# akb825/Cuttlefish

Measured on AMD Instinct MI355X. Metric: Mpixels/s encode, BC7 4096x4096 RGBA8, higher is better.
Workload: dtype u8; 1 GPU; BC7 UNORM Texture::Quality::Normal, one 4096x4096 RGBA8 synthetic photo tile per GPU, resident in HBM; format=BC7, quality=2, blocks_per_launch=1048576, parallelism=surface-per-gpu x1

## Files before the change

cuttlefish_amd/csrc/bc7_encode.hip:

```cpp
#include "cf_device.h"
#include "bc7_packed.h"
#include "bc7_rcp.h"
#include "bc7_roles.h"
#include "bc7_cand.h"

namespace {

#define CF_FRESH_LANE(x) asm volatile("v_mbcnt_lo_u32_b32 %0, -1, 0\n\tv_mbcnt_hi_u32_b32 %0, -1, %0" : "=v"(x))

__device__ __forceinline__ int cf_bperm(int v, uint32_t src)
{
	return __builtin_amdgcn_ds_bpermute((int)(src << 2), v);
}

__device__ const cf_bc7_role_table k_bc7_roles = cf_bc7_make_roles();

__device__ const cf_bc7_cand_table k_bc7_cands = cf_bc7_make_cands();
__device__ const cf_bc7_mask_table k_bc7_masks = cf_bc7_make_masks();

__device__ const cf_bc7_weight_table k_bc7_weights = cf_bc7_make_weights();

__device__ const uint16_t k_part2[64] = CF_BC7_PART2_INIT;

__device__ const uint8_t k_anchor2[64] = {
	15,15,15,15,15,15,15,15, 15,15,15,15,15,15,15,15,
	15, 2, 8, 2, 2, 8, 8,15,  2, 8, 2, 2, 8, 8, 2, 2,
	15,15, 6, 8, 2, 8,15,15,  2, 8, 2, 2, 2,15,15, 6,
	 6, 2, 6, 8,15,15, 2, 2, 15,15,15,15,15, 2, 2,15
};

__device__ const uint32_t k_part3[64] = CF_BC7_PART3_INIT;

__device__ const uint8_t k_anchor3a[64] = {
	 3, 3,15,15, 8, 3,15,15,  8, 8, 6, 6, 6, 5, 3, 3,
	 3, 3, 8,15, 3, 3, 6,10,  5, 8, 8, 6, 8, 5,15,15,
	 8,15, 3, 5, 6,10, 8,15, 15, 3,15, 5,15,15,15,15,
	 3,15, 5, 5, 5, 8, 5,10,  5,10, 8,13,15,12, 3, 3
};

__device__ const uint8_t k_anchor3b[64] = {
	15, 8, 8, 3,15,15, 3, 8, 15,15,15,15,15,15,15, 8,
	15, 8,15, 3,15, 8,15, 8,  3,15, 6,10,15,15,10, 8,
	15, 3,15,10,10, 8, 9,10,  6,15, 8,15, 3, 6, 6, 8,
	15, 3,15,15,15,15,15,15, 15,15,15,15, 3,15,15, 8
};

__device__ __forceinline__ uint32_t part3_mask(uint32_t p3, uint32_t sb)
{
	const uint32_t lo = p3 & 0x55555555u, hi = (p3 >> 1) & 0x55555555u;
	uint32_t x = sb == 0u ? ~(lo | hi) & 0x55555555u : (sb == 1u ? lo & ~hi : (sb == 2u ? hi & ~lo : 0u));
	x = (x | (x >> 1)) & 0x33333333u;
	x = (x | (x >> 2)) & 0x0F0F0F0Fu;
	x = (x | (x >> 4)) & 0x00FF00FFu;
	return (x | (x >> 8)) & 0xFFFFu;
}

struct SubFit {
	uint32_t e0, e1;
	uint32_t q0, q1;
	uint32_t pb;
	uint32_t err;
	uint32_t w[4];
	float nx0[4], nx1[4];
	bool ok;
};

struct Cand {
	uint32_t err, id;
	uint32_t q[6];
	uint32_t pb;
	uint32_t w[4];
	uint32_t w2[4];
};

#define CF_BC7_CAND_WORDS 22
__device__ __forceinline__ void cand_store(uint32_t* slot, const Cand& c)
{
#pragma unroll
	for (int k = 0; k < 6; ++k) slot[k*CF_WG_THREADS] = c.q[k];
	slot[6*CF_WG_THREADS] = c.pb;
#pragma unroll
	for (int k = 0; k < 4; ++k) {
		slot[(7 + k)*CF_WG_THREADS] = c.w[k];
		slot[(11 + k)*CF_WG_THREADS] = c.w2[k];
	}
}

__device__ __forceinline__ uint32_t ub(uint32_t v, int c) { return (v >> (8*c)) & 255u; }
__device__ __forceinline__ float fb(uint32_t v, int c) { return (float)((v >> (8*c)) & 255u); }

__device__ __forceinline__ float clamp255(float x)
{
	return __builtin_amdgcn_fmed3f(x, 0.0f, 255.0f);
}

__device__ const float k_inv_n[17] = {
	__builtin_huge_valf(), 1.0f/1.0f, 1.0f/2.0f, 1.0f/3.0f, 1.0f/4.0f, 1.0f/5.0f, 1.0f/6.0f, 1.0f/7.0f, 1.0f/8.0f,
	1.0f/9.0f, 1.0f/10.0f, 1.0f/11.0f, 1.0f/12.0f, 1.0f/13.0f, 1.0f/14.0f, 1.0f/15.0f, 1.0f/16.0f
};
__device__ __forceinline__ float inv_n(uint32_t n) { return k_inv_n[n < 16u ? n : 16u]; }

// ... 159 lines not shown
}

#ifndef CF_BC7_ABLATE
#define CF_BC7_ABLATE 0
#endif

#ifndef CF_BC7_DIAG
#define CF_BC7_DIAG 0
#endif
#if CF_BC7_DIAG
enum { CF_DIAG_STARTS, CF_DIAG_STARTS_CACHED, CF_DIAG_STARTS_NARROW, CF_DIAG_PERTURB, CF_DIAG_PERTURB_NARROW,
	CF_DIAG_STARTS_NOPB, CF_DIAG_PERTURB_NOPB, CF_DIAG_PERTURB_PPHIT, CF_DIAG_N };
__device__ unsigned long long cf_bc7_diag[CF_DIAG_N];
#define CF_DIAG_COUNT(i, cond) do { uint32_t l_; CF_FRESH_LANE(l_); if (l_ == 0u && (cond)) atomicAdd(&cf_bc7_diag[i], 1ull); } while (0)
#else
#define CF_DIAG_COUNT(i, cond) do { } while (0)
#endif

typedef int cf_int4 __attribute__((ext_vector_type(4)));
template <bool UNITW>
__device__ __forceinline__ void arow_load(const uint32_t* tile, uint32_t boff, uint32_t (&arow)[4])
{
	arow[0] = arow[1] = arow[2] = arow[3] = 0u;
	if (UNITW) {
		uint32_t lane;
		CF_FRESH_LANE(lane);
#pragma unroll
		for (uint32_t r = 0; r < 4u; ++r)
			arow[r] = tile[boff + 4u*r + (lane & 3u)] ^ 0x80808080u;
	}
}

struct LaneFit {
	uint32_t q0, q1, pb, err;
	uint32_t w[4];
};

template <bool UNITW, int NK = 8, int CBSZ = 3>
__device__ __forceinline__ void assign_lsq_lane(const Tex& tx, uint32_t mask, bool m6,
	uint32_t khalf, uint32_t ib, const uint32_t (&yw)[2], uint32_t pp_sum, bool want_lsq, uint32_t fe0, uint32_t fe1, const uint32_t (&arow)[4],
	LaneFit& f, float (&nx0)[4], float (&nx1)[4], float (&hq)[3], bool& ok, uint32_t s01 = 0u, uint32_t s23 = 0u)
{
	constexpr int WBITS = UNITW ? 8 : 7;
	const uint32_t nk = m6 ? 8u : (1u << ib);
	const uint32_t e00 = ub(fe0, 0), e01 = ub(fe0, 1), e02 = ub(fe0, 2), e03 = ub(fe0, 3);
	const uint32_t e10 = ub(fe1, 0), e11 = ub(fe1, 1), e12 = ub(fe1, 2), e13 = ub(fe1, 3);
	uint32_t pal[8], palh[8];
	int base[8];
	uint32_t w03 = 0, w47 = 0;
	const uint32_t* wr = k_bc7_weights.w[weight_row(m6, khalf, ib)];
	w03 = wr[0];
	w47 = NK == 8 ? wr[1] : 0u;
	const uint32_t rsel = tx.rot == 0u ? 0x03020100u : (tx.rot == 1u ? 0x00020103u : (tx.rot == 2u ? 0x01020300u : 0x02030100u));
	const PalLine line = pal_line(__builtin_amdgcn_perm(fe0, fe0, rsel), __builtin_amdgcn_perm(fe1, fe1, rsel));
#pragma unroll
	for (int k = 0; k < NK; ++k) {
		const bool valid = k < 4 || (uint32_t)k < nk;
		const uint32_t w = weight_at(w03, w47, (uint32_t)k);
		const uint32_t iw = 64u - w;
		if (UNITW) {
			pal[k] = pal_at(line, w);
			palh[k] = 0;
			const int B = mfma_entry_base((int)((__builtin_amdgcn_udot4(pal[k], pal[k], 0u, false) << WBITS) | w),
				__builtin_amdgcn_udot4(pal[k], 0x01010101u, 0u, false), WBITS + 1);
			pal[k] ^= 0x80808080u;
			base[k] = valid ? B : CF_BC7_NO_ENTRY;
		} else {
			const uint32_t c0 = (__umul24(iw, e00) + __umul24(w, e10) + 32u) >> 6;
			const uint32_t c1 = (__umul24(iw, e01) + __umul24(w, e11) + 32u) >> 6;
			const uint32_t c2 = (__umul24(iw, e02) + __umul24(w, e12) + 32u) >> 6;
			const uint32_t c3 = (__umul24(iw, e03) + __umul24(w, e13) + 32u) >> 6;
			uint32_t qrg, qba;
			ycc_pairs(c0, c1, c2, c3, qrg, qba);
			pal[k] = pk_mul_u16(qrg, yw[0]);
			palh[k] = pk_mul_u16(qba, yw[1]);
			const uint32_t qq = dot2_u16(pal[k], qrg, dot2_u16(palh[k], qba, 0u));
			const int B = (int)((qq << WBITS) | w);
			base[k] = valid ? B : CF_BC7_NO_ENTRY;
		}
		asm volatile("" : "+v"(base[k]));
	}
	int kfac = -(2 << WBITS);
	asm volatile("" : "+s"(kfac));
	uint32_t err = pp_sum;
	uint32_t wp0 = 0, wp1 = 0, wp2 = 0, wp3 = 0;
#pragma unroll 1
	for (uint32_t r2 = 0; r2 < 4u; r2 += 2u) {
		uint32_t wpair[2];
#pragma unroll
		for (uint32_t h = 0; h < 2u; ++h) {
			const uint32_t r = r2 + h;
			uint32_t raw[4], rawh[4];
			if (UNITW) {
				const uint4 rw = *reinterpret_cast<const uint4*>(tx.tp() + 4u*r);
				raw[0] = rw.x; raw[1] = rw.y; raw[2] = rw.z; raw[3] = rw.w;
				rawh[0] = rawh[1] = rawh[2] = rawh[3] = 0u;
			} else {
				const uint4 ya = *reinterpret_cast<const uint4*>(tx.yc() + 8u*r);
				const uint4 yb = *reinterpret_cast<const uint4*>(tx.yc() + 8u*r + 4u);
				raw[0] = ya.x; raw[1] = ya.z; raw[2] = yb.x; raw[3] = yb.z;
				rawh[0] = ya.y; rawh[1] = ya.w; rawh[2] = yb.y; rawh[3] = yb.w;
			}
			const uint32_t mrow = (mask >> (4u*r)) & 15u;
			uint32_t wrow = 0, krow[4];
			int bestm[4] = {0x7FFFFFFF, 0x7FFFFFFF, 0x7FFFFFFF, 0x7FFFFFFF};
			if (UNITW) {
				const cf_int4 cop = {0, 0, 0, 0};
				const uint32_t aop = r2 == 0u ? (h == 0u ? arow[0] : arow[1]) : (h == 0u ? arow[2] : arow[3]);
#pragma unroll
				for (int k = 0; k < NK; ++k) {
					const cf_int4 d = __builtin_amdgcn_mfma_i32_4x4x4i8((int)aop, (int)pal[k], cop, CBSZ, 0, 0);
					const int v0 = key_min_form(d.x, kfac, base[k]), v1 = key_min_form(d.y, kfac, base[k]);
					const int v2 = key_min_form(d.z, kfac, base[k]), v3 = key_min_form(d.w, kfac, base[k]);
					bestm[0] = v0 < bestm[0] ? v0 : bestm[0]; bestm[1] = v1 < bestm[1] ? v1 : bestm[1];
					bestm[2] = v2 < bestm[2] ? v2 : bestm[2]; bestm[3] = v3 < bestm[3] ? v3 : bestm[3];
				}
			}
#pragma unroll
			for (int j = 0; j < 4; ++j) {
				uint32_t rawj = raw[j];
				if (!UNITW) asm volatile("" : "+v"(rawj), "+v"(wrow));
				uint32_t key;
				{
					int bestk = bestm[j];
					const uint32_t prg = rawj, pba = rawh[j];
#pragma unroll
					for (int k = 0; k < (UNITW ? 0 : NK); ++k) {
						const int dt = (int)dot2_u16(pba, palh[k], dot2_u16(prg, pal[k], 0u));
						const int v = key_min_form(dt, kfac, base[k]);
						bestk = v < bestk ? v : bestk;
					}
					if (NK == 8) {
						const int other = (int)cf_xor1((uint32_t)bestk);
						bestk = (m6 && other < bestk) ? other : bestk;
					}
					key = (uint32_t)bestk;
				}
				key = ((mrow >> j) & 1u) ? key : 0u;
				err += (uint32_t)((int)key >> WBITS);
				if (UNITW) krow[j] = key;
				else wrow |= (key & 127u) << (8*j);
			}
			wpair[h] = UNITW ? key_row_weights(krow[0], krow[1], krow[2], krow[3]) : wrow;
		}
		wp0 = wp2; wp1 = wp3; wp2 = wpair[0]; wp3 = wpair[1];
	}
	f.err = err;
	f.w[0] = wp0; f.w[1] = wp1; f.w[2] = wp2; f.w[3] = wp3;
	uint32_t S = 0, A = 0, B = 0, C = 0, U[4] = {0, 0, 0, 0}, V[4] = {0, 0, 0, 0};
	if (want_lsq) {
#pragma unroll 1
		for (uint32_t r = 0; r < 4u; ++r) {
			const uint32_t wrow = wp0;
			wp0 = wp1; wp1 = wp2; wp2 = wp3; wp3 = wrow;
			uint32_t P[4];
			uint32_t bo = tx.boff;
			asm volatile("" : "+v"(bo));
			planes<true>(tx, *reinterpret_cast<const uint4*>(tx.plan_ + bo + 4u*r), P);
			S = __builtin_amdgcn_udot4(wrow, 0x01010101u, S, false);
			C = __builtin_amdgcn_udot4(wrow, wrow, C, false);
#pragma unroll
			for (int c = 0; c < 4; ++c)
				V[c] = __builtin_amdgcn_udot4(wrow, P[c], V[c], false);
		}
		A = 4096u*(uint32_t)__builtin_popcount(mask) - 128u*S + C;
		B = 64u*S - C;
		U[0] = 64u*(s01 & 0xFFFFu) - V[0]; U[1] = 64u*(s01 >> 16) - V[1];
		U[2] = 64u*(s23 & 0xFFFFu) - V[2]; U[3] = 64u*(s23 >> 16) - V[3];
	}
	const int det = (int)__umul24((uint32_t)__builtin_popcount(mask), C) - (int)__umul24(S, S);
	ok = det > 0;
	const float inv = cf_rcp_ranged(64.0f*(float)(det > 0 ? det : 1));
	const float fA = (float)A, fB = (float)B, fC = (float)C;
#pragma unroll
	for (int c = 0; c < 4; ++c) {
		if ((tx.chmask >> c) & 1u) {
			const float fU = (float)U[c], fV = (float)V[c];
			const float t0 = fB*fV;
			const float n0 = fmaf(fC, fU, -t0);
			const float t1 = fB*fU;
			const float n1 = fmaf(fA, fV, -t1);
			nx0[c] = n0*inv;
			nx1[c] = n1*inv;
		} else {
			nx0[c] = 0.0f;
			nx1[c] = 0.0f;
		}
	}
	hq[0] = fA; hq[1] = fB; hq[2] = fC;
}

__device__ __forceinline__ void refit_window(const float (&xu0)[4], const float (&xu1)[4], const float (&hq)[3],
	uint32_t cb, uint32_t ab, uint32_t pbk, SubFit& f)
{
	const uint32_t S = pbk ? 1u : 0u;
	const uint32_t P0 = f.pb & 1u, P1 = (f.pb >> 1) & 1u;
	const float fA = hq[0], fC = hq[2], fB2 = hq[1] + hq[1];
	const uint32_t tc = cb ? cb + S : 0u, ta = ab ? ab + S : 0u;
	const uint32_t qmaxw = ((1u << cb) - 1u)*0x010101u | (((1u << ab) - 1u) << 24);
	const uint32_t lo0 = f.q0, lo1 = f.q1;
	const uint32_t hi0 = f.q0 ^ qmaxw, hi1 = f.q1 ^ qmaxw;
	uint32_t dw0[3], dw1[3];
	dw0[0] = dequant_word(code_word(((f.q0 | 0x00808080u) - 0x01010101u) & qmaxw, S, P0), tc, ta);
	dw0[1] = f.e0;
	dw0[2] = dequant_word(code_word((f.q0 + 0x01010101u) & qmaxw, S, P0), tc, ta);
	dw1[0] = dequant_word(code_word(((f.q1 | 0x00808080u) - 0x01010101u) & qmaxw, S, P1), tc, ta);
	dw1[1] = f.e1;
	dw1[2] = dequant_word(code_word((f.q1 + 0x01010101u) & qmaxw, S, P1), tc, ta);
	uint32_t pick = 0;
#pragma unroll
	for (int c = 0; c < 4; ++c) {
		const uint32_t bm = 255u << (8*c);
		float dl0[3], dl1[3];
#pragma unroll
		for (int d = 0; d < 3; ++d) {
			dl0[d] = fb(dw0[d], c) - xu0[c];
			dl1[d] = fb(dw1[d], c) - xu1[c];
		}
		dl0[0] = (lo0 & bm) ? dl0[0] : 1.0e18f;
		dl0[2] = (hi0 & bm) ? dl0[2] : 1.0e18f;
		dl1[0] = (lo1 & bm) ? dl1[0] : 1.0e18f;
		dl1[2] = (hi1 & bm) ? dl1[2] : 1.0e18f;
		float best = 3.0e38f;
		uint32_t bi = 0x11u << (8*c);
#pragma unroll
		for (int i = 0; i < 3; ++i) {
			const float d0 = dl0[i];
			float a0 = fA*d0;
			a0 = a0*d0;
			const float cr = fB2*d0;
#pragma unroll
			for (int j = 0; j < 3; ++j) {
				const float d1 = dl1[j];
				float v = fC*d1;
				v = fmaf(v, d1, a0);
				v = fmaf(cr, d1, v);
				const bool take = v < best;
				best = take ? v : best;
				bi = take ? (uint32_t)(i | (j << 4)) << (8*c) : bi;
			}
		}
		pick |= bi;
	}
	const uint32_t nq0 = f.q0 + (pick & 0x03030303u) - 0x01010101u;
	const uint32_t nq1 = f.q1 + ((pick >> 4) & 0x03030303u) - 0x01010101u;
	const uint32_t ne0 = dequant_word(code_word(nq0, S, P0), tc, ta);
	const uint32_t ne1 = dequant_word(code_word(nq1, S, P1), tc, ta);
	f.q0 = nq0; f.q1 = nq1; f.e0 = ne0; f.e1 = ne1;
}

#define CF_BC7_GEO_WORDS 13
// ... 33 lines not shown
		const uint32_t n = (uint32_t)__builtin_popcount(mask);
		uint32_t s[4] = {0, 0, 0, 0};
		uint32_t q00 = 0, q01 = 0, q02 = 0, q03 = 0, q11 = 0, q12 = 0, q13 = 0, q22 = 0, q23 = 0,
			q33 = 0;
		lo = 255u; hi = 0u;
		if (GIVEN && gmode == 3u) {
			uint32_t q[10];
			mom_unpack(gs.W, s, q);
			q00 = q[0]; q01 = q[1]; q02 = q[2]; q03 = q[3]; q11 = q[4]; q12 = q[5]; q13 = q[6]; q22 = q[7]; q23 = q[8]; q33 = q[9];
			lo = gs.lohi & 255u; hi = UNITW ? lohi_hi(gs.lohi) : gs.lohi >> 8;
		} else
#pragma unroll 1
		for (uint32_t r = 0; r < 4u; ++r) {
			uint32_t P[4];
			const uint4 pr = *reinterpret_cast<const uint4*>(tx.pl() + 4u*r);
			planes<true>(tx, pr, P);
			const uint32_t a4 = tx.rot == 0u ? pr.w : (tx.rot == 1u ? pr.x : (tx.rot == 2u ? pr.y : pr.z));
#pragma unroll
			for (int j = 0; j < 4; ++j) {
				const uint32_t a = (a4 >> (8*j)) & 255u;
				lo = a < lo ? a : lo;
				hi = a > hi ? a : hi;
			}
			const uint32_t m4 = bytemask4((mask >> (4u*r)) & 15u);
			const uint32_t M0 = P[0] & m4, M1 = P[1] & m4, M2 = P[2] & m4, M3 = P[3] & m4;
			s[0] = __builtin_amdgcn_udot4(M0, 0x01010101u, s[0], false);
			s[1] = __builtin_amdgcn_udot4(M1, 0x01010101u, s[1], false);
			s[2] = __builtin_amdgcn_udot4(M2, 0x01010101u, s[2], false);
			s[3] = __builtin_amdgcn_udot4(M3, 0x01010101u, s[3], false);
			q00 = __builtin_amdgcn_udot4(M0, P[0], q00, false);
			q01 = __builtin_amdgcn_udot4(M0, P[1], q01, false);
			q02 = __builtin_amdgcn_udot4(M0, P[2], q02, false);
			q03 = __builtin_amdgcn_udot4(M0, P[3], q03, false);
			q11 = __builtin_amdgcn_udot4(M1, P[1], q11, false);
			q12 = __builtin_amdgcn_udot4(M1, P[2], q12, false);
			q13 = __builtin_amdgcn_udot4(M1, P[3], q13, false);
			q22 = __builtin_amdgcn_udot4(M2, P[2], q22, false);
			q23 = __builtin_amdgcn_udot4(M2, P[3], q23, false);
			q33 = __builtin_amdgcn_udot4(M3, P[3], q33, false);
		}
		const float C00 = (float)(int)(__umul24(n, q00) - __umul24(s[0], s[0])), C01 = (float)(int)(__umul24(n, q01) - __umul24(s[0], s[1]));
		const float C02 = (float)(int)(__umul24(n, q02) - __umul24(s[0], s[2])), C03 = (float)(int)(__umul24(n, q03) - __umul24(s[0], s[3]));
		const float C11 = (float)(int)(__umul24(n, q11) - __umul24(s[1], s[1])), C12 = (float)(int)(__umul24(n, q12) - __umul24(s[1], s[2]));
		const float C13 = (float)(int)(__umul24(n, q13) - __umul24(s[1], s[3])), C22 = (float)(int)(__umul24(n, q22) - __umul24(s[2], s[2]));
		const float C23 = (float)(int)(__umul24(n, q23) - __umul24(s[2], s[3])), C33 = (float)(int)(__umul24(n, q33) - __umul24(s[3], s[3]));

		float bestd = C00;
		float v0 = C00, v1 = C01, v2 = C02, v3 = C03;
		if (C11 > bestd) { bestd = C11; v0 = C01; v1 = C11; v2 = C12; v3 = C13; }
		if (C22 > bestd) { bestd = C22; v0 = C02; v1 = C12; v2 = C22; v3 = C23; }
		if (C33 > bestd) { bestd = C33; v0 = C03; v1 = C13; v2 = C23; v3 = C33; }
#pragma unroll
		for (int it = 0; it < 3; ++it) {
			float r0 = C00*v0; r0 = fmaf(C01, v1, r0); r0 = fmaf(C02, v2, r0); r0 = fmaf(C03, v3, r0);
			float r1 = C01*v0; r1 = fmaf(C11, v1, r1); r1 = fmaf(C12, v2, r1); r1 = fmaf(C13, v3, r1);
			float r2 = C02*v0; r2 = fmaf(C12, v1, r2); r2 = fmaf(C22, v2, r2); r2 = fmaf(C23, v3, r2);
			float r3 = C03*v0; r3 = fmaf(C13, v1, r3); r3 = fmaf(C23, v2, r3); r3 = fmaf(C33, v3, r3);
			v0 = r0; v1 = r1; v2 = r2; v3 = r3;
		}
		const float mx = fmaxf(fmaxf(fabsf(v0), fabsf(v1)), fmaxf(fabsf(v2), fabsf(v3)));
#pragma unroll
		for (int c = 0; c < 4; ++c) axis[c] = 0.0f;
		if (mx > 0.0f) {
			const float im = cf_rcp_tested(mx);
			v0 = v0*im; v1 = v1*im; v2 = v2*im; v3 = v3*im;
			float l2 = v0*v0;
			l2 = fmaf(v1, v1, l2);
			l2 = fmaf(v2, v2, l2);
			l2 = fmaf(v3, v3, l2);
			const float is = cf_rcp_ranged(sqrtf(l2));
			axis[0] = v0*is; axis[1] = v1*is; axis[2] = v2*is; axis[3] = v3*is;
		}

		const float in = inv_n(n);
#pragma unroll
		for (int c = 0; c < 4; ++c)
			mean[c] = (float)s[c]*in;
		tmin = 3.0e38f; tmax = -3.0e38f;
#pragma unroll 1
		for (uint32_t r = 0; r < 4u; ++r) {
			const uint4 rw = *reinterpret_cast<const uint4*>(tx.tp() + 4u*r);
			const uint32_t raw[4] = {rw.x, rw.y, rw.z, rw.w};
			const uint32_t mrow = (mask >> (4u*r)) & 15u;
#pragma unroll
			for (int j = 0; j < 4; ++j) {
				const uint32_t p = texel<true>(tx, raw[j]);
				const bool m = (mrow >> j) & 1u;
				float t = axis[0]*(fb(p, 0) - mean[0]);
				t = fmaf(axis[1], fb(p, 1) - mean[1], t);
				t = fmaf(axis[2], fb(p, 2) - mean[2], t);
				t = fmaf(axis[3], fb(p, 3) - mean[3], t);
				tmin = m ? fminf(tmin, t) : tmin;
				tmax = m ? fmaxf(tmax, t) : tmax;
			}
		}
		pp_sum = UNITW ? q00 + q11 + q22 + q33 : ycc_pp_sum(tx, mask, yw);
		if constexpr (UNITW) {
			const uint32_t bias = whole ? lohi_rawsum((GIVEN && gmode == 3u) ? gs.lohi : lohi[tx.boff >> 2])
				: search_bias_part(s[0], s[1], s[2], s[3], n, !(tx.chmask & 8u));
			pp_sum = search_pp_fold(pp_sum, bias);
		}
		s01 = s[0] | (s[1] << 16);
		s23 = s[2] | (s[3] << 16);
		if ((GIVEN ? gmode != 0u : gmode == 1u) && (UNITW ? owner : true)) {
			uint32_t lane;
			CF_FRESH_LANE(lane);
			uint32_t* gc = gbase + lane;
#pragma unroll
			for (int c = 0; c < 4; ++c) {
				gc[c*CF_WG_THREADS] = __float_as_uint(axis[c]);
				gc[(4 + c)*CF_WG_THREADS] = __float_as_uint(mean[c]);
			}
			gc[8*CF_WG_THREADS] = __float_as_uint(tmin);
			gc[9*CF_WG_THREADS] = __float_as_uint(tmax);
			gc[10*CF_WG_THREADS] = lo | (hi << 8);
			gc[11*CF_WG_THREADS] = pp_sum;
		}
	}
	{
		const float d = (tmax - tmin)*frac;
		tmin = tmin + d;
		tmax = tmax - d;
	}
	float x0[4], x1[4];
#pragma unroll
	for (int c = 0; c < 4; ++c) {
		x0[c] = clamp255(fmaf(axis[c], tmin, mean[c]));
		x1[c] = clamp255(fmaf(axis[c], tmax, mean[c]));
	}
	if (scalar) {
		const float flo = (float)lo, fhi = (float)hi;
		const float d = (fhi - flo)*frac;
		x0[0] = 0.0f; x0[1] = 0.0f; x0[2] = 0.0f; x0[3] = clamp255(flo + d);
		x1[0] = 0.0f; x1[1] = 0.0f; x1[2] = 0.0f; x1[3] = clamp255(fhi - d);
	}
	uint32_t geo = cb | (ab << 4) | (pbk << 8) | (ib << 12);
	asm volatile("" : "+v"(geo));
#define G_CB (geo & 15u)
#define G_AB ((geo >> 4) & 15u)
#define G_PBK ((geo >> 8) & 15u)
#define G_IB (geo >> 12)
	SubFit q;
	quantize<UNITW>(x0, x1, G_CB, G_AB, G_PBK, wt, q);
	best.q0 = q.q0; best.q1 = q.q1; best.pb = q.pb;
	bool live;
	float hq[3];
	uint32_t arow[4];
	arow_load<UNITW>(tx.tile_, tx.boff, arow);
	assign_lsq_lane<UNITW, NK, CBSZ>(tx, mask, m6, khalf, G_IB, yw, pp_sum, ITERS > 0u, q.e0, q.e1, arow, best, x0, x1, hq, live, s01, s23);
#pragma unroll 1
	for (uint32_t r = 0; r < ITERS; ++r) {
		LaneFit cur;
		bool ok;
		asm volatile("" : "+v"(geo));
		{
			float c0[4], c1[4];
#pragma unroll
			for (int c = 0; c < 4; ++c) {
				c0[c] = clamp255(x0[c]);
				c1[c] = clamp255(x1[c]);
			}
			quantize<UNITW>(c0, c1, G_CB, G_AB, G_PBK, wt, q);
		}
		if (!(CF_BC7_ABLATE & 8)) refit_window(x0, x1, hq, G_CB, G_AB, G_PBK, q);
		cur.q0 = q.q0; cur.q1 = q.q1; cur.pb = q.pb;
		arow_load<UNITW>(tx.tile_, tx.boff, arow);
		assign_lsq_lane<UNITW, NK, CBSZ>(tx, mask, m6, khalf, G_IB, yw, pp_sum, r + 1u < ITERS, q.e0, q.e1, arow, cur, x0, x1, hq, ok, s01, s23);
		const bool better = live && cur.err < best.err;
		if (better)
			best = cur;
		live = better && ok;
	}
#undef G_CB
#undef G_AB
#undef G_PBK
#undef G_IB
}

__device__ __forceinline__ uint32_t w2i(uint32_t w, uint32_t ib)
{
	return (w*((1u << ib) - 1u) + 32u) >> 6;
}

__device__ __forceinline__ uint4 pack_block_group(const uint32_t* wcol, uint32_t id, uint32_t lane,
	bool pair)
{
	const uint32_t h = lane >> 5, hl = pair ? (lane & 31u) : lane, hbase = pair ? (lane & 32u) : 0u;
	uint32_t mode, part = 0, rot = 0, isel = 0;
	if (id == 0u) mode = 6;
	else if (id < 5u) { mode = 5; rot = id - 1u; }
	else if (id < 13u) { mode = 4; rot = (id - 5u) & 3u; isel = (id - 5u) >> 2; }
	else if (id < 128u) { mode = 1; part = id - 64u; }
	else if (id < 192u) { mode = 3; part = id - 128u; }
	else if (id < 256u) { mode = 0; part = id - 192u; }
	else if (id < 320u) { mode = 2; part = id - 256u; }
	else { mode = 7; part = id - 320u; }
	const uint32_t ns  = (0x21112323u >> (4u*mode)) & 15u;
	const uint32_t pbn = (0x60006664u >> (4u*mode)) & 15u;
	const uint32_t cb  = (0x57757564u >> (4u*mode)) & 15u;
	const uint32_t ab  = (0x57860000u >> (4u*mode)) & 15u;
	const uint32_t pk  = (0x11001021u >> (4u*mode)) & 15u;
	const uint32_t ib  = (0x24222233u >> (4u*mode)) & 15u;
	const uint32_t ib2 = (0x00230000u >> (4u*mode)) & 15u;
	uint32_t ibc = ib, iba = ib2;
	const bool swapsets = mode == 4u && isel != 0u;
	if (swapsets) { ibc = 3u; iba = 2u; }
	const uint32_t p2 = k_part2[part], p3 = k_part3[part];
	uint32_t a1 = 0, a2 = 0;
	if (ns == 2u) a1 = k_anchor2[part];
	else if (ns == 3u) { a1 = k_anchor3a[part]; a2 = k_anchor3b[part]; }

	const uint32_t t = hl & 15u;
	const uint32_t sb = ns == 1u ? 0u : (ns == 2u ? ((p2 >> t) & 1u) : ((p3 >> (2u*t)) & 3u));
	const uint32_t wv = (wcol[(7u + (t >> 2))*CF_WG_THREADS] >> (8u*(t & 3u))) & 255u;
	const uint32_t ws = (wcol[(11u + (t >> 2))*CF_WG_THREADS] >> (8u*(t & 3u))) & 255u;
	uint32_t idxv = w2i(wv, ibc);
	uint32_t idxs = iba ? w2i(ws, iba) : 0u;
	const uint32_t i0 = (uint32_t)cf_bperm((int)idxv, (uint32_t)((int)hbase));
	const uint32_t i1 = (uint32_t)cf_bperm((int)idxv, (uint32_t)((int)(hbase + a1)));
	const uint32_t i2 = (uint32_t)cf_bperm((int)idxv, (uint32_t)((int)(hbase + a2)));
	const uint32_t is0 = (uint32_t)cf_bperm((int)idxs, (uint32_t)((int)hbase));
	const uint32_t sw0 = i0 >> (ibc - 1u);
	const uint32_t sw1 = ns > 1u ? i1 >> (ibc - 1u) : 0u;
	const uint32_t sw2 = ns > 2u ? i2 >> (ibc - 1u) : 0u;
	const uint32_t sws = iba ? is0 >> (iba - 1u) : 0u;
	const uint32_t swmask = sw0 | (sw1 << 1) | (sw2 << 2);
	idxv = ((swmask >> sb) & 1u) ? ((1u << ibc) - 1u) - idxv : idxv;
	idxs = sws ? ((1u << iba) - 1u) - idxs : idxs;

	const uint32_t ne = 2u*ns;
	const uint32_t hdr = mode + 1u + pbn + ((mode == 4u || mode == 5u) ? 2u : 0u) + (mode == 4u ? 1u : 0u);
	const uint32_t base_pb = hdr + ne*(3u*cb + ab);
	const uint32_t npb = pk == 1u ? ne : (pk == 2u ? 2u : 0u);
	const uint32_t baseA = base_pb + npb;
	const uint32_t baseB = baseA + 16u*ib - ns;

	uint32_t w0 = 0, w1 = 0, w2 = 0, w3 = 0;
	const uint32_t npass = pair ? 2u : 1u;
	for (uint32_t pass = 0; pass < npass; ++pass) {
		const uint32_t f = hl + 32u*pass;
		uint32_t val = 0, off = 0;
		bool have = false;
		if (f < 16u) {
			const uint32_t before = (t > 0u ? 1u : 0u) + ((ns >= 2u && t > a1) ? 1u : 0u) +
				((ns == 3u && t > a2) ? 1u : 0u);
			val = swapsets ? idxs : idxv;
			off = baseA + t*ib - before;
			have = true;
		} else if (f < 32u) {
			val = swapsets ? idxv : idxs;
			off = baseB + t*ib2 - (t > 0u ? 1u : 0u);
			have = ib2 != 0u;
		} else if (f < 56u) {
			const uint32_t g = f - 32u;
			const uint32_t ch = g/ne, e = g - ch*ne;
			const uint32_t es = e ^ ((swmask >> (e >> 1)) & 1u);
			const uint32_t qw = wcol[es*CF_WG_THREADS];
			if (ch < 3u) {
				val = (qw >> (8u*ch)) & 255u;
				off = hdr + (ch*ne + e)*cb;
				have = true;
			} else if (ch == 3u && ab) {
				const uint32_t sq = wcol[(4u + ((e ^ sws) & 1u))*CF_WG_THREADS];
				val = (iba ? sq : qw) >> 24;
				off = hdr + 3u*ne*cb + e*ab;
				have = true;
			}
		} else if (f < 62u) {
			const uint32_t e = f - 56u;
			const uint32_t pbw = wcol[6u*CF_WG_THREADS];
			if (pk == 1u && e < ne) {
				val = (pbw >> (e ^ ((swmask >> (e >> 1)) & 1u))) & 1u;
				off = base_pb + e;
				have = true;
			} else if (pk == 2u && e < 2u) {
				val = (pbw >> (2u*e)) & 1u;
				off = base_pb + e;
				have = true;
			}
		} else if (f == 62u) {
			val = (1u << mode) | (part << (mode + 1u)) | (rot << (mode + 1u + pbn)) |
				(isel << (mode + 1u + pbn + 2u));
			if (!(mode == 4u || mode == 5u))
				val = (1u << mode) | (part << (mode + 1u));
			off = 0;
			have = true;
		}
		val = have ? val : 0u;
		const uint32_t wi = off >> 5, sh = off & 31u;
		const unsigned long long vv = (unsigned long long)val << sh;
		const uint32_t lo = (uint32_t)vv, hi = (uint32_t)(vv >> 32);
		w0 |= wi == 0u ? lo : 0u;
		w1 |= wi == 1u ? lo : (wi == 0u ? hi : 0u);
		w2 |= wi == 2u ? lo : (wi == 1u ? hi : 0u);
		w3 |= wi == 3u ? lo : (wi == 2u ? hi : 0u);
	}
	uint4 r;
	r.x = cf_group_or_u32(w0, pair, h);
	r.y = cf_group_or_u32(w1, pair, h);
	r.z = cf_group_or_u32(w2, pair, h);
	r.w = cf_group_or_u32(w3, pair, h);
	return r;
}

struct Moments {
	uint32_t s[4];
	uint32_t q00, q01, q02, q03, q11, q12, q13, q22, q23, q33;
};

#define CF_BC7_MOM_WORDS 10
__device__ __forceinline__ void block_moments_put(const uint32_t* plan, uint32_t* mom, uint32_t t)
{
	const uint32_t b = t >> 4, m = t & 15u;
	if (m >= CF_BC7_MOM_WORDS)
		return;
	const uint32_t ca = m < 4u ? m : (m < 7u ? 0u : (m < 9u ? 1u : 2u));
	const uint32_t cb = m < 4u ? m : (m < 7u ? m - 3u : (m < 9u ? m - 5u : 3u));
	const uint32_t* pb = plan + b*16u;
	const bool opaque = (pb[3] & pb[7] & pb[11] & pb[15]) == 0xFFFFFFFFu;
	uint32_t q = 0, sm = 0;
#pragma unroll
	for (uint32_t r = 0; r < 4u; ++r) {
		const uint32_t A = (opaque && ca == 3u) ? 0u : pb[4u*r + ca], B = (opaque && cb == 3u) ? 0u : pb[4u*r + cb];
		q = __builtin_amdgcn_udot4(A, B, q, false);
		sm = __builtin_amdgcn_udot4(A, 0x01010101u, sm, false);
	}
	mom[b*CF_BC7_MOM_WORDS + m] = m < 4u ? q | (sm << 20) : q;
}

template <bool A4, bool TWO>
__device__ __forceinline__ void moments_rows(const Tex& tx, uint32_t mask1, uint32_t mask2, Moments& a, Moments& b)
{
#pragma unroll
	for (int c = 0; c < 4; ++c) { a.s[c] = 0; b.s[c] = 0; }
	a.q00 = a.q01 = a.q02 = a.q03 = a.q11 = a.q12 = a.q13 = a.q22 = a.q23 = a.q33 = 0;
	b.q00 = b.q01 = b.q02 = b.q03 = b.q11 = b.q12 = b.q13 = b.q22 = b.q23 = b.q33 = 0;
#pragma unroll 1
	for (uint32_t r = 0; r < 4u; ++r) {
		uint32_t P[4];
		planes<false>(tx, *reinterpret_cast<const uint4*>(tx.pl() + 4u*r), P);
#pragma unroll
		for (int k = 0; k < (TWO ? 2 : 1); ++k) {
			Moments& o = k ? b : a;
			const uint32_t m4 = bytemask4(((k ? mask2 : mask1) >> (4u*r)) & 15u);
			const uint32_t M0 = P[0] & m4, M1 = P[1] & m4, M2 = P[2] & m4, M3 = A4 ? P[3] & m4 : 0u;
			o.s[0] = __builtin_amdgcn_udot4(M0, 0x01010101u, o.s[0], false);
			o.s[1] = __builtin_amdgcn_udot4(M1, 0x01010101u, o.s[1], false);
			o.s[2] = __builtin_amdgcn_udot4(M2, 0x01010101u, o.s[2], false);
			if (A4) o.s[3] = __builtin_amdgcn_udot4(M3, 0x01010101u, o.s[3], false);
			o.q00 = __builtin_amdgcn_udot4(M0, P[0], o.q00, false);
			o.q01 = __builtin_amdgcn_udot4(M0, P[1], o.q01, false);
			o.q02 = __builtin_amdgcn_udot4(M0, P[2], o.q02, false);
			if (A4) o.q03 = __builtin_amdgcn_udot4(M0, P[3], o.q03, false);
			o.q11 = __builtin_amdgcn_udot4(M1, P[1], o.q11, false);
			o.q12 = __builtin_amdgcn_udot4(M1, P[2], o.q12, false);
			if (A4) o.q13 = __builtin_amdgcn_udot4(M1, P[3], o.q13, false);
			o.q22 = __builtin_amdgcn_udot4(M2, P[2], o.q22, false);
			if (A4) o.q23 = __builtin_amdgcn_udot4(M2, P[3], o.q23, false);
			if (A4) o.q33 = __builtin_amdgcn_udot4(M3, P[3], o.q33, false);
		}
	}
}

template <bool A4, bool TWO>
__device__ __forceinline__ Moments moments_rest(const uint32_t* tw, const Moments& a, const Moments& b)
{
	Moments o;
	const uint32_t w0 = tw[0], w1 = tw[1], w2 = tw[2], w3 = A4 ? tw[3] : 0u;
#define CF_REST(f, tot) o.f = (tot) - a.f - (TWO ? b.f : 0u)
	CF_REST(s[0], w0 >> 20); CF_REST(s[1], w1 >> 20); CF_REST(s[2], w2 >> 20);
	CF_REST(q00, w0 & 0xFFFFFu); CF_REST(q11, w1 & 0xFFFFFu); CF_REST(q22, w2 & 0xFFFFFu);
// ... 889 lines not shown
```

cuttlefish_amd/csrc/bc7_packed.h:

```cpp
#ifndef CFHIP_BC7_PACKED_H
#define CFHIP_BC7_PACKED_H

#include <stdint.h>

#if defined(__HIPCC__)
#define CF_PK __host__ __device__ __forceinline__
#else
#define CF_PK static inline
#endif
#if defined(__HIP_DEVICE_COMPILE__)
#define CF_PK_MUL24(a, b) __umul24((a), (b))
#else
#define CF_PK_MUL24(a, b) ((a)*(b))
#endif

#if defined(__HIP_DEVICE_COMPILE__)
#define CF_PK_MUL24S(a, b) __mul24((a), (b))
#else
#define CF_PK_MUL24S(a, b) ((a)*(b))
#endif

#define CF_BC7_NO_ENTRY 0x3FFFFFFF
CF_PK int key_min_form(int dt, int m256, int B) { return CF_PK_MUL24S(dt, m256) + B; }


CF_PK int mfma_entry_base(int B, uint32_t sb, int fbits)
{
	return B + (int)(512u << (7 + fbits)) - (int)CF_PK_MUL24(sb, 1u << (7 + fbits));
}

CF_PK uint32_t lohi_pack(uint32_t lohi, uint32_t rawsum) { return lohi | (rawsum << 16); }
CF_PK uint32_t lohi_rawsum(uint32_t w) { return w >> 16; }
CF_PK uint32_t lohi_hi(uint32_t w) { return (w >> 8) & 255u; }
CF_PK uint32_t search_bias_part(uint32_t s0, uint32_t s1, uint32_t s2, uint32_t s3, uint32_t n, bool opaque)
{
	return s0 + s1 + s2 + s3 + (opaque ? CF_PK_MUL24(n, 255u) : 0u);
}
CF_PK uint32_t search_pp_fold(uint32_t pp_sum, uint32_t bias) { return pp_sum - (bias << 8); }

CF_PK uint32_t key_row_weights(uint32_t k0, uint32_t k1, uint32_t k2, uint32_t k3)
{
#if defined(__HIP_DEVICE_COMPILE__)
	return __builtin_amdgcn_perm(k1, k0, 0x0C0C0400u) | __builtin_amdgcn_perm(k3, k2, 0x04000C0Cu);
#else
	return (k0 & 255u) | ((k1 & 255u) << 8) | ((k2 & 255u) << 16) | ((k3 & 255u) << 24);
#endif
}

CF_PK uint32_t dequant1(uint32_t v, uint32_t t)
{
	return CF_PK_MUL24(v, (1u << t) + 1u) >> (2u*t - 8u);
}

CF_PK uint32_t dequant_rgb(uint32_t word, uint32_t t)
{
	const uint32_t c3 = word & 0x00FFFFFFu;
	const uint32_t low = ((1u << (8u - t)) - 1u)*0x010101u;
	return (c3 << (8u - t)) | ((c3 >> (2u*t - 8u)) & low);
}

CF_PK uint32_t dequant_word(uint32_t word, uint32_t tc, uint32_t ta)
{
	const uint32_t coded = (tc ? 0x00FFFFFFu : 0u) | (ta ? 0xFF000000u : 0u);
	return (dequant_rgb(word, tc ? tc : 8u) | (dequant1(word >> 24, ta ? ta : 8u) << 24)) & coded;
}

CF_PK uint32_t code_word(uint32_t qword, uint32_t S, uint32_t P)
{
	return (qword << S) | (P ? 0x01010101u : 0u);
}

CF_PK uint32_t pal_word(uint32_t e0, uint32_t e1, uint32_t w)
{
	const uint32_t iw = 64u - w;
	const uint32_t m = 0x00FF00FFu, half = 0x00200020u;
	const uint32_t rb = CF_PK_MUL24(iw, e0 & m) + CF_PK_MUL24(w, e1 & m) + half;
	const uint32_t ga = CF_PK_MUL24(iw, (e0 >> 8) & m) + CF_PK_MUL24(w, (e1 >> 8) & m) + half;
	return ((rb >> 6) & m) | ((ga << 2) & ~m);
}

struct PalLine { uint32_t rb0, rbd, ga0, gad; };

CF_PK PalLine pal_line(uint32_t e0, uint32_t e1)
{
	const uint32_t m = 0x00FF00FFu, half = 0x00200020u;
	const uint32_t a_rb = e0 & m, a_ga = (e0 >> 8) & m;
	PalLine l;
	l.rb0 = (a_rb << 6) + half; l.rbd = (e1 & m) - a_rb;
	l.ga0 = (a_ga << 6) + half; l.gad = ((e1 >> 8) & m) - a_ga;
	return l;
}

CF_PK uint32_t pal_at(const PalLine& l, uint32_t w)
{
	const uint32_t m = 0x00FF00FFu;
	const uint32_t rb = l.rb0 + w*l.rbd;
	const uint32_t ga = l.ga0 + w*l.gad;
	return ((rb >> 6) & m) | ((ga << 2) & ~m);
}

#define CF_BC7_WEIGHT_ROWS 4u
constexpr uint32_t cf_bc7_weight(uint32_t ib, uint32_t k)
{
	return (k*64u + (((1u << ib) - 1u) >> 1))/((1u << ib) - 1u);
}
struct cf_bc7_weight_table { uint32_t w[CF_BC7_WEIGHT_ROWS][2]; };
constexpr cf_bc7_weight_table cf_bc7_make_weights()
{
	cf_bc7_weight_table t = {};
	for (uint32_t k = 0; k < 8u; ++k) {
		t.w[0][k >> 2] |= (k < 4u ? cf_bc7_weight(2u, k) : 0u) << (8u*(k & 3u));
		t.w[1][k >> 2] |= cf_bc7_weight(3u, k) << (8u*(k & 3u));
		t.w[2][k >> 2] |= cf_bc7_weight(4u, k) << (8u*(k & 3u));
		t.w[3][k >> 2] |= cf_bc7_weight(4u, 8u + k) << (8u*(k & 3u));
	}
	return t;
}
CF_PK uint32_t weight_row(bool m6, uint32_t khalf, uint32_t ib)
{
	return m6 ? 2u + (khalf & 1u) : (ib == 3u ? 1u : 0u);
}
// ... 52 lines not shown
```

Baseline: 3040 Mpixels/s.

## Table-drive BC7 bit packing and streamline unit-weight error and extremes paths

Replaces the per-lane branchy BC7 block bit-packing logic with a precomputed constexpr table of slot descriptors per candidate shape. In the unit-weight path, the error is now formed by summing raw keys and subtracting a weight sum once at the end, instead of shifting each key. The m6 xor-fold is applied once per row on the MFMA results, the LSQ sums loop is unrolled, and min/max projection uses NaN-masked fmin/fmax pairs. These changes aim to cut divergent branches and per-texel ALU work, at the cost of extra constant-memory loads for the pack table and some added register pressure from the unrolling.

```diff
diff --git a/cuttlefish_amd/csrc/bc7_encode.hip b/cuttlefish_amd/csrc/bc7_encode.hip
--- a/cuttlefish_amd/csrc/bc7_encode.hip
+++ b/cuttlefish_amd/csrc/bc7_encode.hip
@@ -3,6 +3,7 @@
 #include "bc7_rcp.h"
 #include "bc7_roles.h"
 #include "bc7_cand.h"
+#include "bc7_pack.h"
 
 namespace {
 
@@ -17,6 +18,7 @@
 
 __device__ const cf_bc7_cand_table k_bc7_cands = cf_bc7_make_cands();
 __device__ const cf_bc7_mask_table k_bc7_masks = cf_bc7_make_masks();
+__device__ const cf_bc7_pack_table k_bc7_pack = cf_bc7_make_pack();
 
 __device__ const cf_bc7_weight_table k_bc7_weights = cf_bc7_make_weights();
 
@@ -342,7 +344,7 @@
 	}
 	int kfac = -(2 << WBITS);
 	asm volatile("" : "+s"(kfac));
-	uint32_t err = pp_sum;
+	uint32_t err = UNITW ? 0u : pp_sum;
 	uint32_t wp0 = 0, wp1 = 0, wp2 = 0, wp3 = 0;
 #pragma unroll 1
 	for (uint32_t r2 = 0; r2 < 4u; r2 += 2u) {
@@ -375,6 +377,15 @@
 					bestm[0] = v0 < bestm[0] ? v0 : bestm[0]; bestm[1] = v1 < bestm[1] ? v1 : bestm[1];
 					bestm[2] = v2 < bestm[2] ? v2 : bestm[2]; bestm[3] = v3 < bestm[3] ? v3 : bestm[3];
 				}
+				if (NK == 8) {
+					if (m6) {
+#pragma unroll
+						for (int j = 0; j < 4; ++j) {
+							const int other = (int)cf_xor1((uint32_t)bestm[j]);
+							bestm[j] = other < bestm[j] ? other : bestm[j];
+						}
+					}
+				}
 			}
 #pragma unroll
 			for (int j = 0; j < 4; ++j) {
@@ -390,14 +401,14 @@
 						const int v = key_min_form(dt, kfac, base[k]);
 						bestk = v < bestk ? v : bestk;
 					}
-					if (NK == 8) {
+					if (NK == 8 && !UNITW) {
 						const int other = (int)cf_xor1((uint32_t)bestk);
 						bestk = (m6 && other < bestk) ? other : bestk;
 					}
 					key = (uint32_t)bestk;
 				}
 				key = ((mrow >> j) & 1u) ? key : 0u;
-				err += (uint32_t)((int)key >> WBITS);
+				err += UNITW ? key : (uint32_t)((int)key >> WBITS);
 				if (UNITW) krow[j] = key;
 				else wrow |= (key & 127u) << (8*j);
 			}
@@ -405,14 +416,15 @@
 		}
 		wp0 = wp2; wp1 = wp3; wp2 = wpair[0]; wp3 = wpair[1];
 	}
-	f.err = err;
+	if (!UNITW) f.err = err;
 	f.w[0] = wp0; f.w[1] = wp1; f.w[2] = wp2; f.w[3] = wp3;
 	uint32_t S = 0, A = 0, B = 0, C = 0, U[4] = {0, 0, 0, 0}, V[4] = {0, 0, 0, 0};
+	constexpr int SUMS_UNROLL = UNITW ? 4 : 1;
 	if (want_lsq) {
-#pragma unroll 1
+#pragma unroll SUMS_UNROLL
 		for (uint32_t r = 0; r < 4u; ++r) {
-			const uint32_t wrow = wp0;
-			wp0 = wp1; wp1 = wp2; wp2 = wp3; wp3 = wrow;
+			const uint32_t wrow = UNITW ? f.w[r] : wp0;
+			if (!UNITW) { wp0 = wp1; wp1 = wp2; wp2 = wp3; wp3 = wrow; }
 			uint32_t P[4];
 			uint32_t bo = tx.boff;
 			asm volatile("" : "+v"(bo));
@@ -427,6 +439,13 @@
 		B = 64u*S - C;
 		U[0] = 64u*(s01 & 0xFFFFu) - V[0]; U[1] = 64u*(s01 >> 16) - V[1];
 		U[2] = 64u*(s23 & 0xFFFFu) - V[2]; U[3] = 64u*(s23 >> 16) - V[3];
+	}
+	if (UNITW) {
+		uint32_t ws = S;
+		if (!want_lsq)
+			ws = __builtin_amdgcn_udot4(f.w[0], 0x01010101u, __builtin_amdgcn_udot4(f.w[1], 0x01010101u,
+				__builtin_amdgcn_udot4(f.w[2], 0x01010101u, __builtin_amdgcn_udot4(f.w[3], 0x01010101u, 0u, false), false), false), false);
+		f.err = search_key_sum_error(pp_sum, err, ws);
 	}
 	const int det = (int)__umul24((uint32_t)__builtin_popcount(mask), C) - (int)__umul24(S, S);
 	ok = det > 0;
@@ -626,16 +645,31 @@
 			const uint4 rw = *reinterpret_cast<const uint4*>(tx.tp() + 4u*r);
 			const uint32_t raw[4] = {rw.x, rw.y, rw.z, rw.w};
 			const uint32_t mrow = (mask >> (4u*r)) & 15u;
-#pragma unroll
-			for (int j = 0; j < 4; ++j) {
-				const uint32_t p = texel<true>(tx, raw[j]);
-				const bool m = (mrow >> j) & 1u;
-				float t = axis[0]*(fb(p, 0) - mean[0]);
-				t = fmaf(axis[1], fb(p, 1) - mean[1], t);
-				t = fmaf(axis[2], fb(p, 2) - mean[2], t);
-				t = fmaf(axis[3], fb(p, 3) - mean[3], t);
-				tmin = m ? fminf(tmin, t) : tmin;
-				tmax = m ? fmaxf(tmax, t) : tmax;
+			if constexpr (UNITW) {
+				float tm[4];
+#pragma unroll
+				for (int j = 0; j < 4; ++j) {
+					const uint32_t p = texel<true>(tx, raw[j]);
+					float t = axis[0]*(fb(p, 0) - mean[0]);
+					t = fmaf(axis[1], fb(p, 1) - mean[1], t);
+					t = fmaf(axis[2], fb(p, 2) - mean[2], t);
+					t = fmaf(axis[3], fb(p, 3) - mean[3], t);
+					tm[j] = proj_or_nan(t, (mrow >> j) & 1u);
+				}
+				proj_extremes2(tmin, tmax, tm[0], tm[1]);
+				proj_extremes2(tmin, tmax, tm[2], tm[3]);
+			} else {
+#pragma unroll
+				for (int j = 0; j < 4; ++j) {
+					const uint32_t p = texel<true>(tx, raw[j]);
+					const bool m = (mrow >> j) & 1u;
+					float t = axis[0]*(fb(p, 0) - mean[0]);
+					t = fmaf(axis[1], fb(p, 1) - mean[1], t);
+					t = fmaf(axis[2], fb(p, 2) - mean[2], t);
+					t = fmaf(axis[3], fb(p, 3) - mean[3], t);
+					tmin = m ? fminf(tmin, t) : tmin;
+					tmax = m ? fmaxf(tmax, t) : tmax;
+				}
 			}
 		}
 		pp_sum = UNITW ? q00 + q11 + q22 + q33 : ycc_pp_sum(tx, mask, yw);
@@ -730,25 +764,12 @@
 	bool pair)
 {
 	const uint32_t h = lane >> 5, hl = pair ? (lane & 31u) : lane, hbase = pair ? (lane & 32u) : 0u;
-	uint32_t mode, part = 0, rot = 0, isel = 0;
-	if (id == 0u) mode = 6;
-	else if (id < 5u) { mode = 5; rot = id - 1u; }
-	else if (id < 13u) { mode = 4; rot = (id - 5u) & 3u; isel = (id - 5u) >> 2; }
-	else if (id < 128u) { mode = 1; part = id - 64u; }
-	else if (id < 192u) { mode = 3; part = id - 128u; }
-	else if (id < 256u) { mode = 0; part = id - 192u; }
-	else if (id < 320u) { mode = 2; part = id - 256u; }
-	else { mode = 7; part = id - 320u; }
-	const uint32_t ns  = (0x21112323u >> (4u*mode)) & 15u;
-	const uint32_t pbn = (0x60006664u >> (4u*mode)) & 15u;
-	const uint32_t cb  = (0x57757564u >> (4u*mode)) & 15u;
-	const uint32_t ab  = (0x57860000u >> (4u*mode)) & 15u;
-	const uint32_t pk  = (0x11001021u >> (4u*mode)) & 15u;
-	const uint32_t ib  = (0x24222233u >> (4u*mode)) & 15u;
-	const uint32_t ib2 = (0x00230000u >> (4u*mode)) & 15u;
-	uint32_t ibc = ib, iba = ib2;
-	const bool swapsets = mode == 4u && isel != 0u;
-	if (swapsets) { ibc = 3u; iba = 2u; }
+	const uint32_t shape = cf_bc7_cand_index(id);
+	const uint32_t* row = k_bc7_pack.w + (shape < CF_CAND_TABLE_N ? shape : CF_CAND_TABLE_N - 1u)*CF_PACK_ROW;
+	const uint32_t cw = row[0];
+	const uint32_t mode = CF_CAND_MODE(cw), ns = CF_CAND_NS(cw);
+	const uint32_t part = ns > 1u ? id & 63u : 0u;
+	const uint32_t ibc = CF_CAND_IB(cw), iba = CF_CAND_IB2(cw);
 	const uint32_t p2 = k_part2[part], p3 = k_part3[part];
 	uint32_t a1 = 0, a2 = 0;
 	if (ns == 2u) a1 = k_anchor2[part];
@@ -771,66 +792,25 @@
 	const uint32_t swmask = sw0 | (sw1 << 1) | (sw2 << 2);
 	idxv = ((swmask >> sb) & 1u) ? ((1u << ibc) - 1u) - idxv : idxv;
 	idxs = sws ? ((1u << iba) - 1u) - idxs : idxs;
-
-	const uint32_t ne = 2u*ns;
-	const uint32_t hdr = mode + 1u + pbn + ((mode == 4u || mode == 5u) ? 2u : 0u) + (mode == 4u ? 1u : 0u);
-	const uint32_t base_pb = hdr + ne*(3u*cb + ab);
-	const uint32_t npb = pk == 1u ? ne : (pk == 2u ? 2u : 0u);
-	const uint32_t baseA = base_pb + npb;
-	const uint32_t baseB = baseA + 16u*ib - ns;
+	const uint32_t swall = swmask | (sws << 3);
+	const uint32_t before = (t > 0u ? 1u : 0u) + ((ns >= 2u && t > a1) ? 1u : 0u) + ((ns == 3u && t > a2) ? 1u : 0u);
+	const uint32_t pbn = cf_bc7_pack_pbn(mode);
+	uint32_t hval = (1u << mode) | (part << (mode + 1u));
+	if (CF_CAND_P45(cw))
+		hval = (1u << mode) | (CF_CAND_ROT(cw) << (mode + 1u + pbn)) | (CF_CAND_ISEL(cw) << (mode + 1u + pbn + 2u));
 
 	uint32_t w0 = 0, w1 = 0, w2 = 0, w3 = 0;
 	const uint32_t npass = pair ? 2u : 1u;
 	for (uint32_t pass = 0; pass < npass; ++pass) {
 		const uint32_t f = hl + 32u*pass;
-		uint32_t val = 0, off = 0;
-		bool have = false;
-		if (f < 16u) {
-			const uint32_t before = (t > 0u ? 1u : 0u) + ((ns >= 2u && t > a1) ? 1u : 0u) +
-				((ns == 3u && t > a2) ? 1u : 0u);
-			val = swapsets ? idxs : idxv;
-			off = baseA + t*ib - before;
-			have = true;
-		} else if (f < 32u) {
-			val = swapsets ? idxv : idxs;
-			off = baseB + t*ib2 - (t > 0u ? 1u : 0u);
-			have = ib2 != 0u;
-		} else if (f < 56u) {
-			const uint32_t g = f - 32u;
-			const uint32_t ch = g/ne, e = g - ch*ne;
-			const uint32_t es = e ^ ((swmask >> (e >> 1)) & 1u);
-			const uint32_t qw = wcol[es*CF_WG_THREADS];
-			if (ch < 3u) {
-				val = (qw >> (8u*ch)) & 255u;
-				off = hdr + (ch*ne + e)*cb;
-				have = true;
-			} else if (ch == 3u && ab) {
-				const uint32_t sq = wcol[(4u + ((e ^ sws) & 1u))*CF_WG_THREADS];
-				val = (iba ? sq : qw) >> 24;
-				off = hdr + 3u*ne*cb + e*ab;
-				have = true;
-			}
-		} else if (f < 62u) {
-			const uint32_t e = f - 56u;
-			const uint32_t pbw = wcol[6u*CF_WG_THREADS];
-			if (pk == 1u && e < ne) {
-				val = (pbw >> (e ^ ((swmask >> (e >> 1)) & 1u))) & 1u;
-				off = base_pb + e;
-				have = true;
-			} else if (pk == 2u && e < 2u) {
-				val = (pbw >> (2u*e)) & 1u;
-				off = base_pb + e;
-				have = true;
-			}
-		} else if (f == 62u) {
-			val = (1u << mode) | (part << (mode + 1u)) | (rot << (mode + 1u + pbn)) |
-				(isel << (mode + 1u + pbn + 2u));
-			if (!(mode == 4u || mode == 5u))
-				val = (1u << mode) | (part << (mode + 1u));
-			off = 0;
-			have = true;
-		}
-		val = have ? val : 0u;
+		const uint32_t s = row[1u + f];
+		const uint32_t kind = CF_PACK_KIND(s);
+		const uint32_t sbit = (swall >> CF_PACK_ORDER(s)) & 1u;
+		const uint32_t cword = wcol[(CF_PACK_WORD(s) ^ (CF_PACK_FLIPW(s) & sbit))*CF_WG_THREADS];
+		const uint32_t cval = (cword >> (CF_PACK_SHIFT(s) ^ (CF_PACK_FLIPS(s) & sbit))) & (CF_PACK_BYTE(s) ? 255u : 1u);
+		uint32_t val = kind == CF_PACK_KIND_COL ? cval : (kind == CF_PACK_KIND_HDR ? hval : (kind == CF_PACK_KIND_IDX1 ? idxv : idxs));
+		val = CF_PACK_HAVE(s) ? val : 0u;
+		const uint32_t off = CF_PACK_OFF(s) - (f < 16u ? before : 0u);
 		const uint32_t wi = off >> 5, sh = off & 31u;
 		const unsigned long long vv = (unsigned long long)val << sh;
 		const uint32_t lo = (uint32_t)vv, hi = (uint32_t)(vv >> 32);
diff --git a/cuttlefish_amd/csrc/bc7_pack.h b/cuttlefish_amd/csrc/bc7_pack.h
--- /dev/null
+++ b/cuttlefish_amd/csrc/bc7_pack.h
@@ -0,0 +1,81 @@
+#ifndef CFHIP_BC7_PACK_H
+#define CFHIP_BC7_PACK_H
+
+#include <stdint.h>
+#include "bc7_cand.h"
+
+#define CF_PACK_OFF(s) ((s) & 255u)
+#define CF_PACK_HAVE(s) (((s) >> 8) & 1u)
+#define CF_PACK_KIND(s) (((s) >> 9) & 3u)
+#define CF_PACK_WORD(s) (((s) >> 11) & 7u)
+#define CF_PACK_SHIFT(s) (((s) >> 14) & 31u)
+#define CF_PACK_BYTE(s) (((s) >> 19) & 1u)
+#define CF_PACK_ORDER(s) (((s) >> 20) & 3u)
+#define CF_PACK_FLIPW(s) (((s) >> 22) & 1u)
+#define CF_PACK_FLIPS(s) (((s) >> 23) & 1u)
+#define CF_PACK_KIND_IDX1 0u
+#define CF_PACK_KIND_IDX2 1u
+#define CF_PACK_KIND_COL 2u
+#define CF_PACK_KIND_HDR 3u
+
+constexpr uint32_t cf_bc7_pack_pbn(uint32_t mode) { return (0x60006664u >> (4u*mode)) & 15u; }
+constexpr uint32_t cf_bc7_pack_ib1(uint32_t mode) { return (0x24222233u >> (4u*mode)) & 15u; }
+constexpr uint32_t cf_bc7_pack_ib2(uint32_t mode) { return (0x00230000u >> (4u*mode)) & 15u; }
+constexpr uint32_t cf_bc7_pack_ab(uint32_t mode) { return (0x57860000u >> (4u*mode)) & 15u; }
+constexpr uint32_t cf_bc7_pack_id_of(uint32_t i) { return i < 13u ? i : (i - 12u)*64u; }
+
+constexpr uint32_t cf_bc7_pack_slot(uint32_t shape, uint32_t f)
+{
+	const uint32_t w = cf_bc7_cand_word(cf_bc7_pack_id_of(shape));
+	const uint32_t mode = CF_CAND_MODE(w);
+	const bool swapsets = mode == 4u && CF_CAND_ISEL(w) != 0u;
+	const uint32_t ns = CF_CAND_NS(w), cb = CF_CAND_CB(w), pk = CF_CAND_PBK(w);
+	const bool p45 = CF_CAND_P45(w) != 0u;
+	const uint32_t ab = cf_bc7_pack_ab(mode), ib = cf_bc7_pack_ib1(mode), ib2 = cf_bc7_pack_ib2(mode);
+	const uint32_t ne = 2u*ns;
+	const uint32_t hdr = mode + 1u + cf_bc7_pack_pbn(mode) + (p45 ? 2u : 0u) + (mode == 4u ? 1u : 0u);
+	const uint32_t base_pb = hdr + ne*(3u*cb + ab);
+	const uint32_t npb = pk == 1u ? ne : (pk == 2u ? 2u : 0u);
+	const uint32_t baseA = base_pb + npb, baseB = baseA + 16u*ib - ns;
+	uint32_t off = 0, have = 0, kind = 0, word = 0, shift = 0, byte = 0, order = 0, flipw = 0, flips = 0;
+	if (f < 16u) {
+		off = baseA + f*ib; have = 1; kind = swapsets ? CF_PACK_KIND_IDX2 : CF_PACK_KIND_IDX1;
+	} else if (f < 32u) {
+		const uint32_t t = f - 16u;
+		off = baseB + t*ib2 - (t > 0u ? 1u : 0u); have = ib2 != 0u ? 1u : 0u; kind = swapsets ? CF_PACK_KIND_IDX1 : CF_PACK_KIND_IDX2;
+	} else if (f < 56u) {
+		const uint32_t g = f - 32u, ch = g/ne, e = g - ch*ne;
+		kind = CF_PACK_KIND_COL; byte = 1;
+		if (ch < 3u) {
+			off = hdr + (ch*ne + e)*cb; have = 1; word = e; shift = 8u*ch; order = e >> 1; flipw = 1;
+		} else if (ch == 3u && ab) {
+			off = hdr + 3u*ne*cb + e*ab; have = 1; shift = 24; flipw = 1;
+			word = p45 ? 4u + e : e; order = p45 ? 3u : e >> 1;
+		}
+	} else if (f < 62u) {
+		const uint32_t e = f - 56u;
+		kind = CF_PACK_KIND_COL; word = 6;
+		if (pk == 1u && e < ne) { off = base_pb + e; have = 1; shift = e; order = e >> 1; flips = 1; }
+		else if (pk == 2u && e < 2u) { off = base_pb + e; have = 1; shift = 2u*e; }
+	} else if (f == 62u) {
+		have = 1; kind = CF_PACK_KIND_HDR;
+	}
+	if (!have)
+		off = kind = word = shift = byte = order = flipw = flips = 0;
+	return off | (have << 8) | (kind << 9) | (word << 11) | (shift << 14) | (byte << 19) | (order << 20) | (flipw << 22) | (flips << 23);
+}
+
+#define CF_PACK_ROW 65u
+struct cf_bc7_pack_table { uint32_t w[CF_CAND_TABLE_N*CF_PACK_ROW]; };
+constexpr cf_bc7_pack_table cf_bc7_make_pack()
+{
+	cf_bc7_pack_table t = {};
+	for (uint32_t i = 0; i < CF_CAND_TABLE_N; ++i) {
+		t.w[i*CF_PACK_ROW] = cf_bc7_cand_word(cf_bc7_pack_id_of(i));
+		for (uint32_t f = 0; f < 64u; ++f)
+			t.w[i*CF_PACK_ROW + 1u + f] = cf_bc7_pack_slot(i, f);
+	}
+	return t;
+}
+
+#endif
diff --git a/cuttlefish_amd/csrc/bc7_packed.h b/cuttlefish_amd/csrc/bc7_packed.h
--- a/cuttlefish_amd/csrc/bc7_packed.h
+++ b/cuttlefish_amd/csrc/bc7_packed.h
@@ -37,6 +37,18 @@
 	return s0 + s1 + s2 + s3 + (opaque ? CF_PK_MUL24(n, 255u) : 0u);
 }
 CF_PK uint32_t search_pp_fold(uint32_t pp_sum, uint32_t bias) { return pp_sum - (bias << 8); }
+
+CF_PK uint32_t search_key_sum_error(uint32_t pp_sum, uint32_t ksum, uint32_t wsum)
+{
+	return pp_sum + (uint32_t)((int)(ksum - wsum) >> 8);
+}
+
+CF_PK float proj_or_nan(float t, bool in_subset) { return in_subset ? t : __builtin_nanf(""); }
+CF_PK void proj_extremes2(float& tmin, float& tmax, float a, float b)
+{
+	tmin = __builtin_fminf(__builtin_fminf(tmin, a), b);
+	tmax = __builtin_fmaxf(__builtin_fmaxf(tmax, a), b);
+}
 
 CF_PK uint32_t key_row_weights(uint32_t k0, uint32_t k1, uint32_t k2, uint32_t k3)
 {
```

Measured after the change: 3127 Mpixels/s, median of 6. 2.9% higher.
